# jcasal-homer/HomerHEVC

Hardware: AMD Instinct MI355X
Metric: encoded frames/sec, 1080p & 2160p YUV420 fixed-QP IPPP, 1/2/4/8 MI355X (higher is better)
Workload: dtype int16; 1 GPU; cfg2-1080p-encode; sequences_per_gpu=256, width=1920, height=1080, wfpp_num_threads=17, qp=32, gop=IPPP intra_period=100

## Files before the change

### homerhevc_amd/csrc/enc/enc_common.h

```cpp
#pragma once
#include "enc_prims.h"
#if !defined(__HIPCC__)
#include <stdio.h>
#include <stdlib.h>
#endif

#if !defined(__HIPCC__) && defined(HENC_TRACE_ENABLE)
#include <stdio.h>
extern "C" FILE *henc_trace_file;
#define HENC_TRACE(...) do { if (henc_trace_file) fprintf(henc_trace_file, __VA_ARGS__); } while (0)
#define HENC_TRACE_PW(e, tag)                                                                                                                      \
	do {                                                                                                                                       \
		if (henc_trace_file) {                                                                                                             \
			unsigned a_[3] = {0, 0, 0};                                                                                                \
			for (int c_ = 0; c_ < 3; c_++) {                                                                                           \
				const int n_ = c_ ? 32 : 64;                                                                                       \
				const pred_t *p_ = c_ ? (e).w->pred_c[c_ - 1] : (e).w->pred_y;                                                     \
				for (int y_ = 0; y_ < n_; y_++)                                                                                    \
					for (int x_ = 0; x_ < n_; x_++) a_[c_] += (unsigned)(p_[y_ * n_ + x_] & 0xffff) * (unsigned)(1 + ((x_ + 3 * y_) & 7)); \
			}                                                                                                                          \
			fprintf(henc_trace_file, "PW %s ctu=%d pred=%u,%u,%u\n", tag, (e).ctu->ctu_number, a_[0], a_[1], a_[2]);                   \
		}                                                                                                                                  \
	} while (0)
#else
#define HENC_TRACE(...) do { } while (0)
#define HENC_TRACE_PW(e, tag) do { } while (0)
#endif

enum { PF_SETUP = 0, PF_MERGE, PF_ME_INT, PF_ME_SUB, PF_PRED_INTER, PF_ENC_INTER, PF_INTRA_SEARCH, PF_INTRA_TU, PF_INTRA_CHROMA, PF_CONSOLIDATE, PF_WAIT, PF_TOTAL, PF_PRIM0, PF_COUNT = PF_PRIM0 + 2 * PP_COUNT + 2 };
#if defined(__HIPCC__) && defined(HENC_PROFILE)
#define HENC_PROF_T0() const unsigned long long prof_t0_ = __builtin_amdgcn_s_memtime()
#if defined(HENC_QPROF)
#define HENC_PROF_ADD(e, cat) do { if ((cat) == PF_TOTAL && (e).prof && threadIdx.x == 0) (e).prof[cat] += __builtin_amdgcn_s_memtime() - prof_t0_; } while (0)
#define HENC_QPROF_T0() unsigned long long qprof_t_ = __builtin_amdgcn_s_memtime()
#define HENC_QPROF_MARK(e, cat) do { const unsigned long long now_ = __builtin_amdgcn_s_memtime(); if ((e).prof && threadIdx.x == 0) (e).prof[cat] += now_ - qprof_t_; qprof_t_ = now_; } while (0)
#define HENC_QPROF_ARG , unsigned long long &qprof_t_
#define HENC_QPROF_PASS , qprof_t_
#else
#define HENC_PROF_ADD(e, cat) do { if ((e).prof && threadIdx.x == 0) (e).prof[cat] += __builtin_amdgcn_s_memtime() - prof_t0_; } while (0)
#endif
#else
#define HENC_PROF_T0() do { } while (0)
#define HENC_PROF_ADD(e, cat) do { } while (0)
#endif
#if !defined(HENC_QPROF_MARK)
#define HENC_QPROF_T0() do { } while (0)
#define HENC_QPROF_MARK(e, cat) do { } while (0)
#define HENC_QPROF_ARG
#define HENC_QPROF_PASS
#endif

namespace henc {

#if defined(__HIPCC__)
extern __constant__ Geo henc_geo_table[NNODES];
#endif
#if defined(__HIP_DEVICE_COMPILE__)
struct GeoTable {
	const Geo *p;
	__device__ __forceinline__ const Geo &operator[](int i) const { return henc_geo_table[__builtin_amdgcn_readfirstlane(i)]; }
	__device__ __forceinline__ const Geo &lane(int i) const { return henc_geo_table[i]; }
};
#else
struct GeoTable {
	const Geo *p;
	HENC_INLINE const Geo &operator[](int i) const { return p[i]; }
	HENC_INLINE const Geo &lane(int i) const { return p[i]; }
};
#endif

constexpr int NHELP_MAX = 3;
constexpr int NODES_RESIDENT = 21, NODES_D3 = 85, NODE_QUAD_D3 = 16, NODE_QUAD_D4 = 64, NODE_SLOTS = NODES_RESIDENT + NODE_QUAD_D3 + NODE_QUAD_D4;
// ... 40 lines not shown
	uint32_t inter_ssq[3];
	int inter_ssq_valid;
	int ctu_x, ctu_y;
	uint32_t nb_ctus;
	unsigned long long *timeline;
	int n_spec_reads, n_ratio_cmp, last_slog;
	int n_stale_pred;
	const uint8_t *rd_ctx;
	int rd_luma_depth;
	uint32_t rd_chroma_state;
	HENC_AT(Node, LDS_OFF_NODES) nodes;
	Node *nodes_fast;
	int node_quad;
	HENC_AT(struct HelperBox, LDS_OFF_BOX) box;
	FastPtr<int16_t> adi_c;
	FastPtr<int16_t> mc_tmp_y;
	int mc_tmp_y_stride;
	FastPtr<int16_t> mc_tmp_c;
	FastPtr<int16_t> scratch_a, scratch_b;
	int hseq[NHELP_MAX];
	int bgseq, bg_node;
};

enum { HJOB_NONE = 0, HJOB_NEW_CTU, HJOB_INTER_TU, HJOB_INTRA_SAD, HJOB_SYNC_CU, HJOB_SSD, HJOB_CHROMA_SEARCH, HJOB_CHROMA_TU, HJOB_QUAD_C, HJOB_QUIT };
#if !defined(HENC_NHELP)
#define HENC_NHELP 1
#endif
constexpr int NHELP = HENC_NHELP;
static_assert(NHELP == NHELP_ && (NHELP == 1 || NHELP == 2), "one helper for both chroma planes, or one per plane");
constexpr int COMP_UV = 3;
struct HelperBox {
	int cmd[NHELP], done[NHELP];
	int job[NHELP];
	int a[NHELP][8];
	uint32_t r[NHELP][8];
	int bg_cmd, bg_done, bg_cancel, bg_ni, bg_depth, bg_mode, bg_bits;
};
#if defined(__HIP_DEVICE_COMPILE__)
static_assert(sizeof(HelperBox) <= LDS_BOX_BYTES && sizeof(Enc) <= LDS_ENC_BYTES, "the places of the mailbox and of the contexts in a worker's LDS");
#endif

template <class G>
HENC_HD void helper_post(const G g, Enc &__restrict__ e, int h, int job, int a0 = 0, int a1 = 0, int a2 = 0, int a3 = 0, int a4 = 0, int a5 = 0)
{
	HENC_ENC_IN_LDS(e);
#if defined(__HIP_DEVICE_COMPILE__)
	HelperBox *b = e.box;
// ... 394 lines not shown
```

### homerhevc_amd/csrc/enc/enc_intra.h

```cpp
#pragma once
#include "enc_common.h"
#include "enc_rdo.h"

namespace henc {

HENC_INLINE int intra_is_filtered(int mode, int inv_depth)
{
	static constexpr int intra_filter[5] = {10, 7, 1, 0, 10};
	const int diff = hmin(habs(mode - HOR_IDX), habs(mode - VER_IDX));
	return (mode != DC_IDX) && (diff > intra_filter[inv_depth - 2]);
}

template <class G>
HENC_HD void node_fill_refs(const G g, Enc &__restrict__ e, int ni, int wnd, int comp, int want_filtered)
{
	HENC_ENC_IN_LDS(e);
	const Geo &q = e.geo[ni];
	const Node &nd = node_of(e, ni);
	const int is_y = comp == COMP_Y;
	const int n = is_y ? q.size : q.size_chroma, x = is_y ? q.x : q.xc, y = is_y ? q.y : q.yc;
	const int pw = is_y ? e.seq->width : e.seq->width >> 1, ph = is_y ? e.seq->height : e.seq->height >> 1;
	const int cx = is_y ? e.ctu_x : e.ctu_x >> 1, cy = is_y ? e.ctu_y : e.ctu_y >> 1;
	const int bl_size = hmin(n, ph - (cy + y + n)), tr_size = hmin(n, pw - (cx + x + n));
	const int st = dec_stride(comp);
// ... 30 lines not shown
}
HENC_INLINE void intra_neighbour_dirs(Enc &__restrict__ e, int ni, int depth, int *dirs, uint16_t *src)
{
	HENC_ENC_IN_LDS(e);
	uint32_t idx = 0;
	CtuPublic *cl = pu_left(e, ni, &idx);
	dirs[0] = dirs[1] = DC_IDX;
	src[0] = src[1] = DC_IDX;
	if (cl == e.ctu) { if (e.w->thread_seen_intra) dirs[0] = read_mode_buff(e, depth, idx, &src[0]); }
	else if (cl) src[0] = (uint16_t)(dirs[0] = cl->pred_mode[idx] == PM_INTRA ? cl->intra_mode[COMP_Y][idx] : DC_IDX);
	CtuPublic *ct = pu_top(e, ni, &idx, 1);
	if (ct == e.ctu) { if (e.w->thread_seen_intra) dirs[1] = read_mode_buff(e, depth, idx, &src[1]); }
	else if (ct) src[1] = (uint16_t)(dirs[1] = ct->pred_mode[idx] == PM_INTRA ? ct->intra_mode[COMP_Y][idx] : DC_IDX);
}

template <class SadsFn, class BitsFn>
HENC_INLINE int intra_search_walk_batched(const int *preds, int rd_fast, double sqrt_lambda, SadsFn &&sads_of, int *best_mode_out, double *best_cost_out, BitsFn &&full_bits_of,
					  int *modes_buf = nullptr, int64_t *sads_buf = nullptr)
{
	static constexpr int search_points[4][5] = {{0, 1, 0, 8, 16}, {2, 10, 16, 22, 30}, {-4, -2, 2, 4, 0}, {-1, 1, 0, 0, 0}};
	static constexpr int num_search_points[4] = {2, 5, 4, 2};
	int best_cu_mode = 0, new_best = 0, min_mode = 0, max_mode = 1, best_bit_cost = 0;
	double best_cost = MAX_COST;
	for (int loop = 0; loop < 4; loop++) {
		if (loop == 1) { best_cu_mode = 2; min_mode = 2; max_mode = 34; }
		int modes_local[5], cnt = 0;
		int64_t sads_local[5];
		int *modes = modes_buf ? modes_buf : modes_local;
		int64_t *sads = sads_buf ? sads_buf : sads_local;
		for (int k = 0; k < num_search_points[loop]; k++) {
			const int mode = best_cu_mode + search_points[loop][k];
			if (mode < min_mode || mode > max_mode) continue;
			modes[cnt++] = mode;
		}
		if (!sads_of(modes, cnt, sads)) return -1;
		for (int k = 0; k < cnt; k++) {
			const int mode = modes[k];
			double cost = (double)(uint32_t)sads[k];
			int bit_cost = 0;
			if (rd_fast == 1) {
				bit_cost = (preds[0] == mode || preds[1] == mode || preds[2] == mode) ? 1 : 12;
				cost += bit_cost * sqrt_lambda;
			} else if (rd_fast == 2) {
				bit_cost = (preds[0] == mode || preds[1] == mode || preds[2] == mode) ? (int)full_bits_of(mode) : 6;
				cost += bit_cost * sqrt_lambda;
			}
			if (cost < best_cost) { best_cost = cost; new_best = mode; best_bit_cost = bit_cost; }
		}
		best_cu_mode = new_best;
	}
	*best_mode_out = best_cu_mode;
	*best_cost_out = best_cost;
	return best_bit_cost;
}
template <class SadFn>
HENC_INLINE int intra_search_walk(const int *preds, int rd_fast, double sqrt_lambda, SadFn &&sad_of, int *best_mode_out, double *best_cost_out)
{
	return intra_search_walk_batched(preds, rd_fast, sqrt_lambda, [&](const int *modes, int cnt, int64_t *sads) -> bool {
		for (int k = 0; k < cnt; k++) {
			sads[k] = sad_of(modes[k]);
			if (sads[k] < 0) return false;
		}
		return true;
	}, best_mode_out, best_cost_out, [](int) { return 0u; });
}

HENC_INLINE uint32_t intra_luma_cost(uint32_t tu_cost, int mode_bits, double correction) { return (uint32_t)(tu_cost + mode_bits * correction + .5); }

template <class G>
HENC_HD int intra_mode_search(const G g, Enc &__restrict__ e, int ni, int depth, int *best_mode_out, double *best_cost_out)
{
	HENC_ENC_IN_LDS(e);
	const Geo &q = e.geo[ni];
	Work &w = *e.w;
	const int n = q.size, curr_depth = q.depth, inv_depth = CFG_MAX_CU_SHIFT - curr_depth;
	node_fill_refs(g, e, ni, depth + 1, COMP_Y, 1);
	int preds[3], dirs[2];
	uint16_t src[2];
	e.rd_luma_depth = curr_depth;
	intra_neighbour_dirs(e, ni, curr_depth, dirs, src);
	mpm_from_dirs(dirs[0], dirs[1], preds);
	const int rd_fast = e.seq->rd_mode == RDM_FAST ? 1 : (rd_full(g, *e.seq) ? 2 : 0);
	SearchLog *lg = nullptr;
	e.last_slog = -1;
	if (rd_fast == 1 && ((src[0] | src[1]) & 0x8000)) {
		if (e.n_spec_reads < MAX_SEARCH_LOGS) {
			lg = e.ctu_g->slog + e.n_spec_reads;
			lg->src[0] = src[0]; lg->src[1] = src[1];
			lg->used[0] = (uint8_t)dirs[0]; lg->used[1] = (uint8_t)dirs[1];
			lg->n = 0;
			lg->has_cmp = 0;
			lg->tu_cost = 0;
			e.last_slog = e.n_spec_reads;
		}
		e.n_spec_reads++;
	}
	const src_t *orig = w.curr_y + q.y * CTU_STRIDE_Y + q.x;
	return intra_search_walk_batched(preds, rd_fast, e.f->sqrt_lambda, [&](const int *modes, int cnt, int64_t *sads) -> bool {
		for (int k0 = 0; k0 < cnt;) {
			const int take = HENC_HELPERS(e) ? hmin(1 + NHELP, cnt - k0) : 1, mine = k0 + take - 1;
			for (int j = 0; j < take - 1; j++) helper_post(g, e, j, HJOB_INTRA_SAD, ni, n, modes[k0 + j], intra_is_filtered(modes[k0 + j], inv_depth));
			{
				const int mode = modes[mine], filt = intra_is_filtered(mode, inv_depth);
				sads[mine] = (int64_t)intra_predict_sad(g, (pred_t *)nullptr, 0, orig, CTU_STRIDE_Y, filt ? w.adi_f : w.adi, n, mode, 1);
			}
			for (int j = 0; j < take - 1; j++) {
				helper_wait(g, e, j);
				sads[k0 + j] = (int64_t)e.box->r[j][0];
			}
			k0 += take;
		}
		if (lg)
			for (int k = 0; k < cnt; k++) {
				lg->mode[lg->n] = (uint8_t)modes[k];
				lg->sad[lg->n] = (uint32_t)sads[k];
				lg->n++;
			}
		return true;
	}, best_mode_out, best_cost_out, [&](int mode) { return rd_bits_luma_mode_in_preds(e, mode, preds); }, w.srch_modes, w.srch_sads);
}

template <class G>
HENC_HD void set_intra_info_buffs(const G g, Enc &__restrict__ e, int depth, int ni)
{
	HENC_ENC_IN_LDS(e);
	const Geo &q = e.geo[ni];
	const Node &nd = node_of(e, ni);
	Work &w = *e.w;
	for (int i = g.tid; i < q.num_part; i += g.n) {
		w.cbf_buffs[COMP_Y][depth][q.abs_index + i] = (uint8_t)nd.intra_cbf[COMP_Y];
		w.tr_idx_buffs[depth][q.abs_index + i] = (uint8_t)nd.intra_tr_idx;
		w.intra_mode_buffs[COMP_Y][depth][q.abs_index + i] = (uint8_t)nd.intra_mode[COMP_Y];
	}
	g.sync();
}

template <class G>
HENC_HD uint32_t encode_intra_tu(const G g, Enc &__restrict__ e, int ni, int depth, int cu_mode, int part_size_type, int *curr_sum)
{
	HENC_ENC_IN_LDS(e);
	const Geo &q = e.geo[ni];
	Node &nd = node_of(e, ni);
// ... 202 lines not shown
		return intra_luma_cost(tn.cost, bitcost_cu_mode, correction);
	}
	return tn.cost;
}

HENC_INLINE void chroma_dir_list(int *list, int luma_mode)
{
	list[0] = PLANAR_IDX; list[1] = VER_IDX; list[2] = HOR_IDX; list[3] = DC_IDX; list[4] = DM_CHROMA_IDX;
#pragma unroll
	for (int i = 0; i < 4; i++)
		if (luma_mode == list[i]) list[i] = 34;
}

template <class G>
HENC_WALK_FN HENC_HD void chroma_search_comp(const G g, Enc &__restrict__ e, int curr, int c, const int *cand, uint32_t *sads)
{
	HENC_ENC_IN_LDS(e);
	Work &w = *e.w;
	const Geo &q = e.geo[curr];
	const int n = q.size_chroma;
	pred_t *pred = pred_ptr(w, c) + q.yc * CTU_STRIDE_C + q.xc;
	const src_t *orig = curr_ptr(w, c) + q.yc * CTU_STRIDE_C + q.xc;
	node_fill_refs(g, e, curr, NWND - 1, c, 0);
	for (int mi = 0; mi < 5; mi++) sads[mi] = intra_predict_sad(g, pred, CTU_STRIDE_C, orig, CTU_STRIDE_C, e.adi_c, n, cand[mi], 0);
}
template <class G>
HENC_HD int chroma_tu_comp(const G g, Enc &__restrict__ e, int curr, int c, int cu_mode, int scan_mode, int shifts, int per, int rem, int *curr_sum_out)
{
	HENC_ENC_IN_LDS(e);
	Work &w = *e.w;
	const Geo &q = e.geo[curr];
	const int n = q.size_chroma, curr_depth = q.depth, qwnd = NWND - 1, dwnd = NWND - 1;
	pred_t *pred = pred_ptr(w, c) + q.yc * CTU_STRIDE_C + q.xc;
	const src_t *orig = curr_ptr(w, c) + q.yc * CTU_STRIDE_C + q.xc;
	int16_t *quant = tq_ptr(w, qwnd, c) + ((q.abs_index << 4) >> 2), *iquant = iq_slot(w, c, (q.abs_index << 4) >> 2, e.on_helper);
	int16_t *dec = dec_ptr(w, dwnd, c) + q.yc * DEC_STRIDE_C + q.xc;
	node_fill_refs(g, e, curr, dwnd, c, 0);
	intra_predict(g, pred, CTU_STRIDE_C, e.adi_c, n, cu_mode, 0);
	tr_forward(g, HENC_FT(e), e.T, orig, CTU_STRIDE_C, pred, CTU_STRIDE_C, e.scratch_a, e.scratch_b, n, 0);
	const int curr_sum = quantize(g, HENC_FT(e), e.T, e.scratch_a, iquant, e.scratch_b, scan_mode, curr_depth, c, 1, e.f->slice_type == SLICE_I, e.seq->sign_hiding, n, per, rem);
	const int cbfv = ((curr_sum ? 1 : 0) << (shifts & 255)) | ((curr_sum ? 1 : 0) << (shifts >> 8));
	bytes_set(g, &w.cbf_chroma[c - 1][q.abs_index], cbfv, q.num_part);
	uint32_t raw;
	if (curr_sum) {
		lin_copy_nosync(g, iquant, quant, n * n);
		dequantize(g, HENC_FT(e), e.T, iquant, iquant, curr_depth, c, 1, n, per, rem);
		tr_inverse(g, HENC_FT(e), e.T, e.scratch_b, n, iquant, e.scratch_a, n, 0);
// ... 32 lines not shown
	} else parent = e.geo[curr].parent;
	const int luma_mode = w.intra_mode_buffs[COMP_Y][depth][e.geo[curr].abs_index];
#if !defined(__HIPCC__)
	if (luma_mode & MODE_TOKEN) { fprintf(stderr, "encode_intra_chroma: inherited luma mode\n"); abort(); }
#endif
	int mode_list[5];
	chroma_dir_list(mode_list, luma_mode);
	if (e.geo[curr].size_chroma == 2) {
		curr = parent;
		parent = e.geo[curr].parent;
	}
	int best_modes[3] = {0, 0, 0};
	double best_costs[3] = {1.7e+308, 1.7e+308, 1.7e+308};
	uint32_t best_bits[3] = {0, 0, 0};
	{
		const Geo &q = e.geo[curr];
		const int n = q.size_chroma;
		uint32_t sad_u[5], sad_v[5];
		int cand[5];
#pragma unroll
		for (int mi = 0; mi < 5; mi++) cand[mi] = mode_list[mi] == DM_CHROMA_IDX ? luma_mode : mode_list[mi];
		if (HENC_HELPERS(e)) {
			helper_post(g, e, 0, HJOB_CHROMA_SEARCH, curr, COMP_U, cand[0] | (cand[1] << 8) | (cand[2] << 16) | (cand[3] << 24), cand[4]);
			chroma_search_comp(g, e, curr, COMP_V, cand, sad_v);
			helper_wait(g, e, 0);
#pragma unroll
			for (int mi = 0; mi < 5; mi++) sad_u[mi] = e.box->r[0][mi];
		} else {
			chroma_search_comp(g, e, curr, COMP_U, cand, sad_u);
			chroma_search_comp(g, e, curr, COMP_V, cand, sad_v);
		}
#pragma unroll
		for (int mi = 0; mi < 5; mi++) {
			uint32_t distortion = sad_u[mi], cost = distortion;
			distortion += sad_v[mi];
			cost += distortion;
			uint32_t bit_cost = mode_list[mi] == DM_CHROMA_IDX ? 1 : 12;
			if (rd_full(g, S)) {
				const Geo &sq = e.geo[curr];
				bytes_set(g, &w.intra_mode_buffs[COMP_CHR][depth][sq.abs_index], mode_list[mi], sq.num_part);
				RdViews &rv = rd_views_of(e);
				rd_make_views(g, e, rv, depth, depth, nullptr, nullptr, depth, nullptr, nullptr, nullptr);
				bit_cost = rd_bits_chroma_mode(e, rv.v, curr);
			}
			cost += (uint32_t)(bit_cost * e.f->sqrt_lambda + .5);
			int um = mode_list[mi];
			double uc = cost;
			uint32_t ub = bit_cost;
#pragma unroll
			for (int i = 0; i < 3; i++)
				if (best_costs[i] > uc) {
					const int am = best_modes[i]; const double ac = best_costs[i]; const uint32_t ab = best_bits[i];
					best_costs[i] = uc; best_modes[i] = um; best_bits[i] = ub;
// ... 131 lines not shown
```

### homerhevc_amd/csrc/enc/enc_prims.h

```cpp
#pragma once
#include "enc_types.h"
#include "../tables_layout.h"

enum { PP_SAD = 0, PP_SSD, PP_BLK, PP_FILLREF, PP_ADIFILT, PP_INTRAPRED, PP_INTERP, PP_TRF, PP_TRI, PP_QUANT, PP_DEQUANT, PP_CAND, PP_SYNC, PP_INFO, PP_CTU_IO, PP_HWAIT, PP_COUNT };
#if defined(__HIPCC__) && defined(HENC_PROFILE)
extern __shared__ __align__(16) unsigned char henc_lds[];
#define HENC_LDS_PROF_OFFSET 43008
#define PRIM_T0() const unsigned long long prim_t0_ = __builtin_amdgcn_s_memtime()
#define PRIM_END(cat) do { if (threadIdx.x == 0) { unsigned long long *pp_ = (unsigned long long *)(henc_lds + HENC_LDS_PROF_OFFSET); pp_[cat] += __builtin_amdgcn_s_memtime() - prim_t0_; pp_[PP_COUNT + (cat)]++; } } while (0)
#else
#define PRIM_T0() do { } while (0)
#define PRIM_END(cat) do { } while (0)
#endif

namespace henc {

HENC_INLINE int ilog2i(int n)
{
	return n <= 1 ? 0 : 32 - __builtin_clz((unsigned)(n - 1));
}
HENC_INLINE void split_rc(int k, int w, int lw, int *r, int *c)
{
	if ((w & (w - 1)) == 0) { *r = k >> lw; *c = k & (w - 1); }
	else { *r = k / w; *c = k - *r * w; }
// ... 560 lines not shown
	PRIM_END(PP_INTRAPRED);
}

template <class G, class S, class P>
HENC_PRIM uint32_t intra_predict_sad(const G g, P *pred, int ps, const S *orig, int os, const int16_t *adi, int n, int mode, int is_luma)
{
	PRIM_T0();
	if constexpr (G::n == 64) { mode = uni(mode); n = uni(n); is_luma = uni(is_luma); }
	const IntraPredictor p = intra_setup(g, adi, n, mode, is_luma);
	const int l = p.shift;
	uint32_t acc = 0;
	#pragma unroll 4
	for (int k = g.tid; k < n * n; k += g.n) {
		const int j = k >> l, i = k & (n - 1);
		const int v = intra_sample(p, j, i);
		if (pred) pred[j * ps + i] = (P)v;
		acc += (uint32_t)habs((int16_t)(orig[j * os + i] - (int16_t)v));
	}
	const uint32_t s = g.sum(acc);
	g.sync();
	{ const auto prim_ret_ = s; PRIM_END(PP_INTRAPRED); return prim_ret_; }
}

HENC_INLINE void luma_tap_row(int f, int *c)
{
	const int t[4][8] = {{0, 0, 0, 64, 0, 0, 0, 0}, {-1, 4, -10, 58, 17, -5, 1, 0}, {-1, 4, -11, 40, 40, -11, 4, -1}, {0, 1, -5, 17, 58, -10, 4, -1}};
	for (int k = 0; k < 8; k++) c[k] = t[f][k];
}
HENC_INLINE void chroma_tap_row(int f, int *c)
{
	const int t[8][4] = {{0, 64, 0, 0}, {-2, 58, 10, -2}, {-4, 54, 16, -2}, {-6, 46, 28, -4}, {-4, 36, 36, -4}, {-4, 28, 46, -6}, {-2, 16, 54, -4}, {-2, 10, 58, -2}};
	for (int k = 0; k < 4; k++) c[k] = t[f][k];
}

template <int NT, class G>
HENC_PRIM void interp_stage(const G g, const int16_t *src, int ss, int16_t *dst, int ds, int fraction, int w, int h, int vert, int first, int last)
{
	PRIM_T0();
	if (NT == 4 && w < 4 && fraction == 0) { g.sync(); PRIM_END(PP_INTERP); return; }
	const int lw = ilog2i(w);
	if ((w & 3) != 0 || (fraction != 0 && w * h < 4 * G::n && G::n > 1)) {
		int c8[8];
		if (NT == 8) luma_tap_row(fraction, c8);
		else chroma_tap_row(fraction, c8);
		const int rs = vert ? ss : 1;
		int shift = 6, offset;
// ... 807 lines not shown
```

### homerhevc_amd/csrc/enc/enc_types.h

```cpp
#pragma once
#include "enc_platform.h"

namespace henc {

enum { COMP_Y = 0, COMP_U = 1, COMP_V = 2, COMP_CHR = 1 };
enum { PM_INTER = 0, PM_INTRA = 1 };
enum { PART_2Nx2N = 0, PART_NxN = 3 };
enum { SLICE_B = 0, SLICE_P = 1, SLICE_I = 2 };
enum { RDM_DIST_ONLY = 0, RDM_FULL = 1, RDM_FAST = 2 };
enum { ME_PEL = 1, ME_HALF = 2, ME_QUARTER = 4 };
enum { PLANAR_IDX = 0, DC_IDX = 1, HOR_IDX = 10, VER_IDX = 26, DM_CHROMA_IDX = 36, REG_DCT = 65535 };
enum { SCAN_ZIGZAG = 0, SCAN_HOR = 1, SCAN_VER = 2, SCAN_DIAG = 3 };

constexpr int NPART = 256;
constexpr int NNODES = 341;
constexpr int NDEPTH = 5;
constexpr int NWND = 7;
constexpr uint32_t MAX_COST = 0xffffffffu / 8;

constexpr int MAX_SEARCH_LOGS = 192, MAX_RATIO_CMP = 96;
constexpr int POST_MAX_ROWS = 128;
constexpr int HENC_MAX_STEPS = 192;
constexpr int MODE_TOKEN = 0x80;

// ... 157 lines not shown
#if defined(__HIPCC__)
	int16_t iq_y[32 * 32], iq_c[HENC_IQ_SLOTS][32 * 32];
#else
	int16_t iq_y[64 * 64], iq_c[2][32 * 32];
#endif
	uint8_t cbf_buffs[3][NDEPTH][NPART];
	uint8_t intra_mode_buffs[2][NDEPTH][NPART];
#if defined(__HIPCC__)
	const uint8_t (*mode_in)[NDEPTH][NPART];
#else
	uint8_t mode_in[2][NDEPTH][NPART];
#endif
	uint8_t tr_idx_buffs[NDEPTH][NPART];
	uint8_t cbf_chroma[2][NPART];
	int16_t adi[264], adi_f[264];
	int16_t pred_aux[TU_SCRATCH];
	int16_t delta_u[TU_SCRATCH];
#if !defined(__HIPCC__)
	int16_t sub_tmp[(64 + 8) * 72];
#endif
	MvCandList amvp, merge_cands, search_cands;
	uint32_t rsplit[11];
	uint32_t pad_rsplit_;
	alignas(8) int64_t srch_sads[5];
	int32_t srch_modes[6];
#if !defined(__HIPCC__)
	uint8_t nodes_fast_store[52 * (21 + 16 + 64) + 16];
#endif
	HENC_GLOBAL_PTR(WorkSlow) slow;
	int32_t thread_seen_intra;
#if !defined(__HIPCC__)
	struct WorkRd *rd_store;
#endif
};
struct WorkRd {
	uint8_t rd_pred_depth[NPART], rd_part_size[NPART], rd_pred_mode[NPART], rd_luma_modes[NPART];
	uint8_t rd_ctx_work[RD_CTX_BYTES];
	EntScratch rd_ent;
	alignas(8) unsigned char rd_views[512];
};

HENC_INLINE int16_t *wnd_y(int16_t *base) { return base; }

HENC_INLINE int16_t *dec_ptr(Work &w, int wnd, int comp)
{
	return (int16_t *)(comp == COMP_Y ? w.slow->dec_y[wnd] + DEC_ORG_Y : w.slow->dec_c[wnd][comp - 1] + DEC_ORG_C);
}
HENC_INLINE int dec_stride(int comp) { return comp == COMP_Y ? DEC_STRIDE_Y : DEC_STRIDE_C; }
// ... 18 lines not shown
```

### homerhevc_amd/csrc/k_encode.hip

```cpp
#define HENC_TU_OPERANDS_IN_LDS 1
#include <stddef.h>
#include <stdlib.h>
#include <algorithm>
#include <chrono>
#include <mutex>
#include <condition_variable>
#include <new>
#include <string>
#include <thread>
#include <vector>

#include <type_traits>
#include "common.h"
#include "enc/enc_sched.h"
#include "enc/enc_host.h"
#include "enc/enc_post.h"
#include "picture_io.h"

using namespace henc;

int hmr_subpel_plane_on(hipStream_t stream, int comp, const int16_t *pic, int stride, int rows, uint8_t *out);
int hmr_subpel_planes_on(hipStream_t stream, const int16_t *pic_y, const int16_t *pic_u, const int16_t *pic_v, int stride_y, int rows_y, int stride_c, int rows_c, uint8_t *out_y,
			 uint8_t *out_u, uint8_t *out_v);

// ... 139 lines not shown
			const Geo &q = e.geo[a[0]];
			if (a[1] == COMP_UV) {
				const int n = q.size_chroma, l = ilog2i(n);
				uint32_t acc[2] = {0, 0};
				for (int i = g.tid * 4; i < n * n; i += 64 * 4) {
					const int o = q.yc * 32 + q.xc + (i >> l) * 32 + (i & (n - 1));
#pragma unroll
					for (int c = 0; c < 2; c++) {
						const S4 va = ld4(e.w->curr_c[c] + o), vb = ld4(e.w->pred_c[c] + o);
#pragma unroll
						for (int k = 0; k < 4; k++) { const int32_t dd = (int16_t)(va.v[k] - vb.v[k]); acc[c] += (uint32_t)(dd * dd); }
					}
				}
				r0 = g.sum(acc[0]);
				r1 = g.sum(acc[1]);
			} else {
				const int c = a[1] - 1;
				r0 = blk_ssd(g, e.w->curr_c[c] + q.yc * 32 + q.xc, 32, e.w->pred_c[c] + q.yc * 32 + q.xc, 32, q.size_chroma);
			}
			break;
		}
		case HJOB_CHROMA_SEARCH: {
			const int cand[5] = {a[2] & 255, (a[2] >> 8) & 255, (a[2] >> 16) & 255, (a[2] >> 24) & 255, a[3]};
			uint32_t sads[5];
			chroma_search_comp(g, e, a[0], a[1], cand, sads);
			g.sync();
			if (g.tid == 0)
				for (int k = 0; k < 5; k++) box->r[h][k] = sads[k];
			break;
		}
		case HJOB_CHROMA_TU: {
			int cs = 0;
			r0 = (uint32_t)chroma_tu_comp(g, e, a[0], a[1], a[2], a[3], a[4], a[5] & 255, a[5] >> 8, &cs);
			r1 = (uint32_t)cs;
			break;
		}
#if defined(HENC_QUAD)
		case HJOB_QUAD_C:
			quad_chroma_job(g, e, a[0], a[1]);
			break;
#endif
		case HJOB_INTRA_SAD: {
			const Geo &q = e.geo[a[0]];
			r0 = intra_predict_sad(g, (pred_t *)nullptr, 0, e.w->curr_y + q.y * CTU_STRIDE_Y + q.x, CTU_STRIDE_Y, a[3] ? e.w->adi_f : e.w->adi, a[1], a[2], 1);
			break;
		}
		default: break;
		}
		g.sync();
		if (g.tid == 0) {
			if (job != HJOB_CHROMA_SEARCH) { box->r[h][0] = r0; box->r[h][1] = r1; box->r[h][2] = r2; box->r[h][3] = r3; box->r[h][4] = r4; box->r[h][5] = r5; }
			__hip_atomic_store(&box->done[h], seq, __ATOMIC_RELEASE, __HIP_MEMORY_SCOPE_WORKGROUP);
		}
	}
	return true;
}

__device__ __attribute__((noinline)) bool helper_serve_out(HelperBox *box, int h, int16_t *scratch, const WaveGrp g, int seq) { return helper_serve(box, h, scratch, g, seq); }

__device__ __attribute__((noinline)) bool helper_bg_search(HelperBox *box, int h, int16_t *scratch, const WaveGrp g, int &seq, int bgseq)
{
	extern __shared__ __align__(16) uint8_t lds[];
	Enc &e = *(Enc *)(lds + LDS_OFF_ENC + (1 + h) * LDS_ENC_BYTES);
	HENC_ENC_IN_LDS(e);
	const int ni = uni(box->bg_ni), depth = uni(box->bg_depth);
	const Geo &q = e.geo[ni];
	const int n = q.size, curr_depth = q.depth, inv_depth = CFG_MAX_CU_SHIFT - curr_depth;
	bool quit = false;
	int best_mode = 0, bits = -1;
	double best_cost = 0;
	if (__hip_atomic_load(&box->bg_cancel, __ATOMIC_ACQUIRE, __HIP_MEMORY_SCOPE_WORKGROUP) != bgseq) {
		node_fill_refs(g, e, ni, depth + 1, COMP_Y, 1);
		int preds[3], dirs[2];
		uint16_t src[2];
// ... 634 lines not shown
```

### homerhevc_amd/csrc/k_primtest.hip

```cpp
#include <stdlib.h>
#include <string.h>
#include <vector>

#include "common.h"
#include "enc/enc_prims.h"

using namespace henc;

hmr_gpu_ctx *hmr_default_ctx();

namespace {

enum { PT_SAD = 1, PT_SSD, PT_PREDICT, PT_RECONST, PT_VARIANCE, PT_INTRA_PRED, PT_FILL_REFS, PT_ADI_FILTER, PT_TRANSFORM, PT_ITRANSFORM, PT_QUANT, PT_INV_QUANT };

struct PtArgs {
	int op, bytes;
	int p[12];
	long off[6];
};

int g_bytes = 0;

__global__ __launch_bounds__(64) void k_primtest(PtArgs a, int16_t *arena, uint8_t *arena8, const DevTables *T, uint32_t *ret)
{
	const WaveGrp g{(int)threadIdx.x};
	const int *p = a.p;
	auto A = [&](int k) { return arena + a.off[k]; };
	auto B = [&](int k) { return arena8 + a.off[k]; };
	uint32_t r = 0;
	switch (a.op) {
	case PT_SAD: r = blk_sad(g, A(0), p[0], A(1), p[1], p[2]); break;
	case PT_SSD: r = a.bytes ? blk_ssd(g, B(0), p[0], B(1), p[1], p[2]) : blk_ssd(g, A(0), p[0], A(1), p[1], p[2]); break;
	case PT_PREDICT:
		if (a.bytes) blk_predict(g, B(0), p[0], B(1), p[1], A(2), p[2], p[3]);
		else blk_predict(g, A(0), p[0], A(1), p[1], A(2), p[2], p[3]);
		break;
	case PT_RECONST: {
		const int16_t *res = p[1] ? A(1) : nullptr;
		if (a.bytes) blk_reconst(g, B(0), p[0], res, p[1], A(2), p[2], p[3]);
		else blk_reconst(g, A(0), p[0], res, p[1], A(2), p[2], p[3]);
		break;
	}
	case PT_VARIANCE: r = a.bytes ? blk_modified_variance(g, B(0), p[1], p[0], p[2]) : blk_modified_variance(g, A(0), p[1], p[0], p[2]); break;
	case PT_INTRA_PRED:
		if (a.bytes) {
			intra_predict(g, B(0), p[0], A(1), p[1], p[2], p[3]);
			g.sync();
			for (int i = g.tid; i < p[1] * p[1]; i += 64) A(0)[(i / p[1]) * p[0] + i % p[1]] = B(0)[(i / p[1]) * p[0] + i % p[1]];
		} else intra_predict(g, A(0), p[0], A(1), p[1], p[2], p[3]);
		break;
	case PT_FILL_REFS: intra_fill_refs(g, A(0), p[0], p[1], p[2], p[3], p[4], p[5], p[6], p[7], A(1)); break;
	case PT_ADI_FILTER: intra_adi_filter(g, A(0), A(1), p[0], p[1]); break;
	case PT_TRANSFORM:
		if (a.bytes) tr_forward(g, (const FastTables *)nullptr, T, B(0), p[0], B(3), p[0], A(1), A(2), p[1], p[2]);
		else tr_forward(g, (const FastTables *)nullptr, T, A(0), p[0], A(3), p[0], A(1), A(2), p[1], p[2]);
		break;
	case PT_ITRANSFORM: tr_inverse(g, (const FastTables *)nullptr, T, A(0), p[0], A(1), A(2), p[1], p[2]); break;
	case PT_QUANT: r = (uint32_t)quantize(g, (const FastTables *)nullptr, T, A(0), A(1), A(2), p[0], p[1], p[2], p[3], p[4], p[5], p[6], p[7], p[8]); break;
	case PT_INV_QUANT: dequantize(g, (const FastTables *)nullptr, T, A(0), A(1), p[0], p[1], p[2], p[3], p[4], p[5]); break;
	default: break;
	}
	g.sync();
	if (g.tid == 0) *ret = r;
}

struct Operand {
	const int16_t *in;
	int16_t *out;
	size_t elems;
};

uint32_t run(int op, const int *p, int np, Operand *ops, int nops)
{
	hmr_gpu_ctx *c = hmr_default_ctx();
	if (!c) { fprintf(stderr, "hmr_gpu_prim_*: no device\n"); abort(); }
	PtArgs a;
	memset(&a, 0, sizeof a);
	a.op = op;
	a.bytes = g_bytes;
	for (int i = 0; i < np; i++) a.p[i] = p[i];
	size_t total = 0;
	for (int k = 0; k < nops; k++) {
// ... 140 lines not shown
	}
	Operand ops[4] = {{block, nullptr, span(block_stride, n, n)}, {nullptr, coeff, (size_t)n * n}, {nullptr, nullptr, (size_t)n * n}, {nullptr, nullptr, span(block_stride, n, n)}};
	const int p[3] = {block_stride, n, is_dst};
	run(PT_TRANSFORM, p, 3, ops, 4);
}
void hmr_gpu_prim_itransform(int16_t *block, int16_t *coeff, int block_stride, int n, int is_dst)
{
	Operand ops[3] = {{block, block, span(block_stride, n, n)}, {coeff, nullptr, (size_t)n * n}, {nullptr, nullptr, (size_t)n * n}};
	const int p[3] = {block_stride, n, is_dst};
	run(PT_ITRANSFORM, p, 3, ops, 3);
}
void hmr_gpu_prim_quant(int16_t *src, int16_t *dst, int16_t *delta_u, int scan_mode, int depth, int comp, int is_intra, int slice_is_intra, int sign_hiding, int *ac_sum,
			int cu_size, int per, int rem)
{
	Operand ops[3] = {{src, nullptr, (size_t)cu_size * cu_size}, {nullptr, dst, (size_t)cu_size * cu_size}, {nullptr, delta_u, (size_t)cu_size * cu_size}};
	const int p[9] = {scan_mode, depth, comp, is_intra, slice_is_intra, sign_hiding, cu_size, per, rem};
	*ac_sum = (int)run(PT_QUANT, p, 9, ops, 3);
}
void hmr_gpu_prim_inv_quant(int16_t *src, int16_t *dst, int depth, int comp, int is_intra, int cu_size, int per, int rem)
{
	Operand ops[2] = {{src, nullptr, (size_t)cu_size * cu_size}, {nullptr, dst, (size_t)cu_size * cu_size}};
	const int p[6] = {depth, comp, is_intra, cu_size, per, rem};
	run(PT_INV_QUANT, p, 6, ops, 2);
}
int hmr_gpu_prim_multi_sad(int maxc, const uint8_t *src, const uint8_t *plane, size_t plane_bytes, const int64_t *cand_off, int ncalls, int stride, int n, uint32_t *out)
{
	if (!src || !plane || !cand_off || !out || ncalls < 1 || ncalls > 65536 || (maxc != 4 && maxc != 8 && maxc != 9) || (n != 8 && n != 16 && n != 32 && n != 64) || stride < 1) {
		hmr_set_error("hmr_gpu_prim_multi_sad: maxc 4 / 8 / 9, n 8 / 16 / 32 / 64, a stride of at least 1, 1 .. 65536 lists");
		return HMR_GPU_ERR_ARG;
	}
	for (int i = 0; i < ncalls * maxc; i++) {
		const int64_t o = cand_off[i];
		if (o == -1) continue;
		if (o < 0 || (uint64_t)o + (uint64_t)(n - 1) * (uint64_t)stride + (uint64_t)n > (uint64_t)plane_bytes) {
			hmr_set_error("hmr_gpu_prim_multi_sad: candidate %d of list %d does not lie inside the plane", i % maxc, i / maxc);
			return HMR_GPU_ERR_ARG;
		}
	}
	hmr_gpu_ctx *c = hmr_default_ctx();
	if (!c) { hmr_set_error("hmr_gpu_prim_multi_sad: no device"); return HMR_GPU_ERR_NO_DEVICE; }
	HIP_TRY(hipSetDevice(c->device));
	struct Bufs {
		void *p[4] = {nullptr, nullptr, nullptr, nullptr};
		~Bufs() { for (void *q : p) if (q) (void)hipFree(q); }
	} b;
	const size_t nres = (size_t)ncalls * maxc;
// ... 17 lines not shown
```

### include/homer_gpu.h

```cpp
#ifndef HOMER_GPU_H
#define HOMER_GPU_H

#include <stddef.h>
#include <stdint.h>

#ifdef __cplusplus
extern "C" {
#endif

typedef struct hmr_gpu_ctx hmr_gpu_ctx;

enum hmr_gpu_status {
	HMR_GPU_OK = 0,
	HMR_GPU_ERR_NO_DEVICE = -1,
	HMR_GPU_ERR_HIP = -2,
	HMR_GPU_ERR_ARG = -3,
	HMR_GPU_ERR_NOMEM = -4
};


int hmr_gpu_create(hmr_gpu_ctx **out, int device, void *stream);
void hmr_gpu_destroy(hmr_gpu_ctx *ctx);
const char *hmr_gpu_last_error(void);
int hmr_gpu_sync(hmr_gpu_ctx *ctx);
// ... 439 lines not shown

int hmr_gpu_subpel_planes(hmr_gpu_ctx *ctx, const int16_t *pic_y, const int16_t *pic_u, const int16_t *pic_v, int stride_y, int rows_y, int stride_c, int rows_c,
			  uint8_t *out_y, uint8_t *out_u, uint8_t *out_v);

int hmr_gpu_probe_valu_issue(hmr_gpu_ctx *ctx, int waves_per_simd, int dependent, double *wave_instr_per_s, double *ms);
int hmr_gpu_probe_issue(hmr_gpu_ctx *ctx, int op, int waves_per_simd, int dependent, double *wave_instr_per_s, double *ms);

void hmr_gpu_prim_bytes(int on);
uint32_t hmr_gpu_prim_sad(int16_t *src, uint32_t src_stride, int16_t *pred, uint32_t pred_stride, int size);
uint32_t hmr_gpu_prim_ssd16b(int16_t *src, uint32_t src_stride, int16_t *pred, uint32_t pred_stride, int size);
void hmr_gpu_prim_predict(int16_t *orig, int orig_stride, int16_t *pred, int pred_stride, int16_t *residual, int residual_stride, int size);
void hmr_gpu_prim_reconst(int16_t *pred, int pred_stride, int16_t *residual, int residual_stride, int16_t *decoded, int decoded_stride, int size);
uint32_t hmr_gpu_prim_modified_variance(int16_t *p, int size, int stride, int modif);
void hmr_gpu_prim_intra_planar(int16_t *prediction, int pred_stride, int16_t *adi_pred_buff, int adi_size, int cu_size);
void hmr_gpu_prim_intra_angular(int16_t *prediction, int pred_stride, int16_t *adi_pred_buff, int adi_size, int cu_size, int cu_mode, int is_luma);
void hmr_gpu_prim_fill_reference_samples(int16_t *decoded_corner, int stride, int n, int left, int top, int bottom_left, int top_right, int bl_size, int tr_size, int16_t *adi);
void hmr_gpu_prim_adi_filter(int16_t *adi, int16_t *out, int adi_size, int n, int strong_enabled);
void hmr_gpu_prim_transform(int16_t *block, int16_t *coeff, int block_stride, int n, int is_dst);
void hmr_gpu_prim_itransform(int16_t *block, int16_t *coeff, int block_stride, int n, int is_dst);
void hmr_gpu_prim_quant(int16_t *src, int16_t *dst, int16_t *delta_u, int scan_mode, int depth, int comp, int is_intra, int slice_is_intra, int sign_hiding, int *ac_sum,
			int cu_size, int per, int rem);
void hmr_gpu_prim_inv_quant(int16_t *src, int16_t *dst, int depth, int comp, int is_intra, int cu_size, int per, int rem);
int hmr_gpu_prim_multi_sad(int maxc, const uint8_t *src, const uint8_t *plane, size_t plane_bytes, const int64_t *cand_off, int ncalls, int stride, int n, uint32_t *out);

enum hmr_gpu_walk_step { HMR_GPU_WALK_QUAD8_Y = 1, HMR_GPU_WALK_QUAD8_C, HMR_GPU_WALK_QUAD16_Y, HMR_GPU_WALK_QUAD16_C, HMR_GPU_WALK_TU, HMR_GPU_WALK_TU_PAIR };
typedef struct hmr_gpu_walk_case {
	int32_t step, node, comp, one_slot;
	int32_t qp, ctu_x, ctu_y, slice_type;
	int32_t sign_hiding, chroma_qp_offset, stride_y, stride_c;
	int32_t mv[4][2];
	double avg_dist, chroma_weight;
	int64_t sub_y, sub_c[2], curr, pred;
} hmr_gpu_walk_case;
typedef struct hmr_gpu_walk_out {
	uint32_t dist[4][3];
	int32_t sum[4][3];
	uint32_t raw[4][3], cbf[4][3];
	uint32_t stray, reserved[15];
	uint8_t pred[4][256];
	int16_t rec[4][256], lv[4][256];
} hmr_gpu_walk_out;
int hmr_gpu_walk_forms(const hmr_gpu_walk_case *cases, int ncases, const uint8_t *arena, size_t arena_bytes, hmr_gpu_walk_out *out);

#ifdef __cplusplus
}
#endif
// ... 2 lines not shown
```

Baseline: 493.1 frames/s.

## Batch intra direction SADs into one multi-mode primitive and split across helper

Adds a multi-direction intra predict+SAD primitive that keeps the source block in registers and reduces all directions at the end, rather than one predict/SAD with its own reduction and sync per mode. The luma search merges the first two search stages into one batch of up to seven modes and sends half the batch to a helper wave in a single mailbox post, replacing the per-mode helper handshakes. Chroma search uses the same batched primitive. The cost is speculative SAD work for the second-stage modes, higher register pressure from the accumulators, and extra profiling macros and a test entry point.

New measurement: 487.5 frames/s. -1.1%, worse.

```diff
diff --git a/homerhevc_amd/csrc/enc/enc_common.h b/homerhevc_amd/csrc/enc/enc_common.h
--- a/homerhevc_amd/csrc/enc/enc_common.h
+++ b/homerhevc_amd/csrc/enc/enc_common.h
@@ -33,7 +33,14 @@
 #if defined(HENC_QPROF)
 #define HENC_PROF_ADD(e, cat) do { if ((cat) == PF_TOTAL && (e).prof && threadIdx.x == 0) (e).prof[cat] += __builtin_amdgcn_s_memtime() - prof_t0_; } while (0)
 #define HENC_QPROF_T0() unsigned long long qprof_t_ = __builtin_amdgcn_s_memtime()
-#define HENC_QPROF_MARK(e, cat) do { const unsigned long long now_ = __builtin_amdgcn_s_memtime(); if ((e).prof && threadIdx.x == 0) (e).prof[cat] += now_ - qprof_t_; qprof_t_ = now_; } while (0)
+#define HENC_QPROF_MARK_(e, cat) do { const unsigned long long now_ = __builtin_amdgcn_s_memtime(); if ((e).prof && threadIdx.x == 0) (e).prof[cat] += now_ - qprof_t_; qprof_t_ = now_; } while (0)
+#if HENC_QPROF == 2
+#define HENC_QPROF_MARK(e, cat) do { (void)qprof_t_; } while (0)
+#define HENC_IQPROF_MARK(e, cat) HENC_QPROF_MARK_(e, cat)
+#define HENC_IQPROF_COUNT(e, cat, k) do { if ((e).prof && threadIdx.x == 0) (e).prof[cat] += (k); } while (0)
+#else
+#define HENC_QPROF_MARK(e, cat) HENC_QPROF_MARK_(e, cat)
+#endif
 #define HENC_QPROF_ARG , unsigned long long &qprof_t_
 #define HENC_QPROF_PASS , qprof_t_
 #else
@@ -48,6 +55,10 @@
 #define HENC_QPROF_MARK(e, cat) do { } while (0)
 #define HENC_QPROF_ARG
 #define HENC_QPROF_PASS
+#endif
+#if !defined(HENC_IQPROF_MARK)
+#define HENC_IQPROF_MARK(e, cat) do { } while (0)
+#define HENC_IQPROF_COUNT(e, cat, k) do { } while (0)
 #endif
 
 namespace henc {
@@ -134,7 +145,8 @@
 	int bgseq, bg_node;
 };
 
-enum { HJOB_NONE = 0, HJOB_NEW_CTU, HJOB_INTER_TU, HJOB_INTRA_SAD, HJOB_SYNC_CU, HJOB_SSD, HJOB_CHROMA_SEARCH, HJOB_CHROMA_TU, HJOB_QUAD_C, HJOB_QUIT };
+enum { HJOB_NONE = 0, HJOB_NEW_CTU, HJOB_INTER_TU, HJOB_INTRA_SAD, HJOB_SYNC_CU, HJOB_SSD, HJOB_CHROMA_SEARCH, HJOB_CHROMA_TU, HJOB_QUAD_C, HJOB_QUIT,
+       HJOB_INTRA_SADS };
 #if !defined(HENC_NHELP)
 #define HENC_NHELP 1
 #endif
diff --git a/homerhevc_amd/csrc/enc/enc_intra.h b/homerhevc_amd/csrc/enc/enc_intra.h
--- a/homerhevc_amd/csrc/enc/enc_intra.h
+++ b/homerhevc_amd/csrc/enc/enc_intra.h
@@ -76,19 +76,27 @@
 	static constexpr int num_search_points[4] = {2, 5, 4, 2};
 	int best_cu_mode = 0, new_best = 0, min_mode = 0, max_mode = 1, best_bit_cost = 0;
 	double best_cost = MAX_COST;
+	int modes_local[7], cnt = 0, first = 0;
+	int64_t sads_local[7];
+	int *modes = modes_buf ? modes_buf : modes_local;
+	int64_t *sads = sads_buf ? sads_buf : sads_local;
 	for (int loop = 0; loop < 4; loop++) {
 		if (loop == 1) { best_cu_mode = 2; min_mode = 2; max_mode = 34; }
-		int modes_local[5], cnt = 0;
-		int64_t sads_local[5];
-		int *modes = modes_buf ? modes_buf : modes_local;
-		int64_t *sads = sads_buf ? sads_buf : sads_local;
-		for (int k = 0; k < num_search_points[loop]; k++) {
-			const int mode = best_cu_mode + search_points[loop][k];
-			if (mode < min_mode || mode > max_mode) continue;
-			modes[cnt++] = mode;
-		}
-		if (!sads_of(modes, cnt, sads)) return -1;
-		for (int k = 0; k < cnt; k++) {
+		if (loop == 1) { first = cnt; cnt += num_search_points[1]; }
+		else {
+			first = cnt = 0;
+			for (int k = 0; k < num_search_points[loop]; k++) {
+				const int mode = best_cu_mode + search_points[loop][k];
+				if (mode < min_mode || mode > max_mode) continue;
+				modes[cnt++] = mode;
+			}
+			const int mine = cnt;
+			if (loop == 0)
+				for (int k = 0; k < num_search_points[1]; k++) modes[cnt++] = 2 + search_points[1][k];
+			if (!sads_of(modes, cnt, sads)) return -1;
+			cnt = mine;
+		}
+		for (int k = first; k < cnt; k++) {
 			const int mode = modes[k];
 			double cost = (double)(uint32_t)sads[k];
 			int bit_cost = 0;
@@ -128,7 +136,9 @@
 	const Geo &q = e.geo[ni];
 	Work &w = *e.w;
 	const int n = q.size, curr_depth = q.depth, inv_depth = CFG_MAX_CU_SHIFT - curr_depth;
+	HENC_QPROF_T0();
 	node_fill_refs(g, e, ni, depth + 1, COMP_Y, 1);
+	HENC_IQPROF_MARK(e, 1);
 	int preds[3], dirs[2];
 	uint16_t src[2];
 	e.rd_luma_depth = curr_depth;
@@ -150,20 +160,32 @@
 		e.n_spec_reads++;
 	}
 	const src_t *orig = w.curr_y + q.y * CTU_STRIDE_Y + q.x;
-	return intra_search_walk_batched(preds, rd_fast, e.f->sqrt_lambda, [&](const int *modes, int cnt, int64_t *sads) -> bool {
-		for (int k0 = 0; k0 < cnt;) {
-			const int take = HENC_HELPERS(e) ? hmin(1 + NHELP, cnt - k0) : 1, mine = k0 + take - 1;
-			for (int j = 0; j < take - 1; j++) helper_post(g, e, j, HJOB_INTRA_SAD, ni, n, modes[k0 + j], intra_is_filtered(modes[k0 + j], inv_depth));
-			{
-				const int mode = modes[mine], filt = intra_is_filtered(mode, inv_depth);
-				sads[mine] = (int64_t)intra_predict_sad(g, (pred_t *)nullptr, 0, orig, CTU_STRIDE_Y, filt ? w.adi_f : w.adi, n, mode, 1);
-			}
-			for (int j = 0; j < take - 1; j++) {
-				helper_wait(g, e, j);
-				sads[k0 + j] = (int64_t)e.box->r[j][0];
-			}
-			k0 += take;
-		}
+	HENC_IQPROF_MARK(e, 2);
+	HENC_IQPROF_COUNT(e, 7, 1);
+	const int bits = intra_search_walk_batched(preds, rd_fast, e.f->sqrt_lambda, [&](const int *modes, int cnt, int64_t *sads) -> bool {
+		#if defined(HENC_INTRA_SPLIT_FIRST_ONLY)
+		const int theirs = HENC_HELPERS(e) && cnt == INTRA_SADS_MAX ? cnt >> 1 : 0, mine = cnt - theirs;
+#else
+		const int theirs = HENC_HELPERS(e) ? cnt >> 1 : 0, mine = cnt - theirs;
+#endif
+		HENC_IQPROF_MARK(e, 6);
+		HENC_IQPROF_COUNT(e, 8, 1);
+		HENC_IQPROF_COUNT(e, 9, cnt);
+		uint64_t list = 0;
+#pragma unroll
+		for (int k = 0; k < INTRA_SADS_MAX; k++) {
+			const int mode = modes[k];
+			list |= (uint64_t)(k < cnt ? intra_sads_entry(mode, intra_is_filtered(mode, inv_depth)) : 0u) << (8 * k);
+		}
+		if (theirs) helper_post(g, e, 0, HJOB_INTRA_SADS, ni, n, (int)(uint32_t)(list >> (8 * mine)), theirs);
+		HENC_IQPROF_MARK(e, 3);
+		intra_predict_sads(g, (pred_t *)nullptr, 0, orig, CTU_STRIDE_Y, (const int16_t *)w.adi, (const int16_t *)w.adi_f, n, list, mine, 1, sads);
+		HENC_IQPROF_MARK(e, 4);
+		if (theirs) {
+			helper_wait(g, e, 0);
+			for (int j = 0; j < theirs; j++) sads[mine + j] = (int64_t)e.box->r[0][j];
+		}
+		HENC_IQPROF_MARK(e, 5);
 		if (lg)
 			for (int k = 0; k < cnt; k++) {
 				lg->mode[lg->n] = (uint8_t)modes[k];
@@ -172,6 +194,8 @@
 			}
 		return true;
 	}, best_mode_out, best_cost_out, [&](int mode) { return rd_bits_luma_mode_in_preds(e, mode, preds); }, w.srch_modes, w.srch_sads);
+	HENC_IQPROF_MARK(e, 6);
+	return bits;
 }
 
 template <class G>
@@ -420,7 +444,10 @@
 	pred_t *pred = pred_ptr(w, c) + q.yc * CTU_STRIDE_C + q.xc;
 	const src_t *orig = curr_ptr(w, c) + q.yc * CTU_STRIDE_C + q.xc;
 	node_fill_refs(g, e, curr, NWND - 1, c, 0);
-	for (int mi = 0; mi < 5; mi++) sads[mi] = intra_predict_sad(g, pred, CTU_STRIDE_C, orig, CTU_STRIDE_C, e.adi_c, n, cand[mi], 0);
+	uint64_t list = 0;
+#pragma unroll
+	for (int mi = 0; mi < 5; mi++) list |= (uint64_t)intra_sads_entry(cand[mi], 0) << (8 * mi);
+	intra_predict_sads(g, pred, CTU_STRIDE_C, orig, CTU_STRIDE_C, (const int16_t *)e.adi_c, (const int16_t *)e.adi_c, n, list, 5, 0, sads);
 }
 template <class G>
 HENC_HD int chroma_tu_comp(const G g, Enc &__restrict__ e, int curr, int c, int cu_mode, int scan_mode, int shifts, int per, int rem, int *curr_sum_out)
@@ -499,13 +526,17 @@
 		for (int mi = 0; mi < 5; mi++) cand[mi] = mode_list[mi] == DM_CHROMA_IDX ? luma_mode : mode_list[mi];
 		if (HENC_HELPERS(e)) {
 			helper_post(g, e, 0, HJOB_CHROMA_SEARCH, curr, COMP_U, cand[0] | (cand[1] << 8) | (cand[2] << 16) | (cand[3] << 24), cand[4]);
-			chroma_search_comp(g, e, curr, COMP_V, cand, sad_v);
+			chroma_search_comp(g, e, curr, COMP_V, cand, w.srch_out);
 			helper_wait(g, e, 0);
 #pragma unroll
-			for (int mi = 0; mi < 5; mi++) sad_u[mi] = e.box->r[0][mi];
+			for (int mi = 0; mi < 5; mi++) { sad_u[mi] = e.box->r[0][mi]; sad_v[mi] = w.srch_out[mi]; }
 		} else {
-			chroma_search_comp(g, e, curr, COMP_U, cand, sad_u);
-			chroma_search_comp(g, e, curr, COMP_V, cand, sad_v);
+			chroma_search_comp(g, e, curr, COMP_U, cand, w.srch_out);
+#pragma unroll
+			for (int mi = 0; mi < 5; mi++) sad_u[mi] = w.srch_out[mi];
+			chroma_search_comp(g, e, curr, COMP_V, cand, w.srch_out);
+#pragma unroll
+			for (int mi = 0; mi < 5; mi++) sad_v[mi] = w.srch_out[mi];
 		}
 #pragma unroll
 		for (int mi = 0; mi < 5; mi++) {
diff --git a/homerhevc_amd/csrc/enc/enc_prims.h b/homerhevc_amd/csrc/enc/enc_prims.h
--- a/homerhevc_amd/csrc/enc/enc_prims.h
+++ b/homerhevc_amd/csrc/enc/enc_prims.h
@@ -606,6 +606,65 @@
 	{ const auto prim_ret_ = s; PRIM_END(PP_INTRAPRED); return prim_ret_; }
 }
 
+constexpr int INTRA_SADS_MAX = 7;
+HENC_INLINE uint32_t intra_sads_entry(int mode, int filtered) { return (uint32_t)mode | (filtered ? 128u : 0u); }
+template <class G, class S, class P, class O>
+#if defined(__HIPCC__) && defined(HENC_INTRA_SADS_OUTLINE)
+__device__ __attribute__((noinline))
+#elif defined(__HIPCC__)
+__device__ __forceinline__
+#else
+inline
+#endif
+void intra_predict_sads(const G g, P *pred, int ps, const S *orig, int os, const int16_t *adi, const int16_t *adi_f, int n, uint64_t list, int cnt, int is_luma, O *out)
+{
+	PRIM_T0();
+	uint32_t list_lo = (uint32_t)list, list_hi = (uint32_t)(list >> 32);
+	if constexpr (G::n == 64) {
+		pred = uni_ptr(pred); orig = uni_ptr(orig); adi = uni_ptr(adi); adi_f = uni_ptr(adi_f); out = uni_ptr(out);
+		ps = uni(ps); os = uni(os); n = uni(n); cnt = uni(cnt); is_luma = uni(is_luma); list_lo = uni(list_lo); list_hi = uni(list_hi);
+	}
+	HENC_OP_IN_LDS(orig); HENC_OP_IN_LDS(adi); HENC_OP_IN_LDS(adi_f); HENC_OP_IN_LDS(out);
+	cnt = hmin(cnt, INTRA_SADS_MAX);
+	const int l = ilog2i(n), total = n * n;
+	const bool kept = total <= 4 * G::n;
+	uint64_t src4 = 0;
+	if (kept) {
+#pragma unroll
+		for (int t = 0; t < 4; t++) {
+			const int k = g.tid + t * G::n;
+			if (k < total) src4 |= (uint64_t)(uint16_t)orig[(k >> l) * os + (k & (n - 1))] << (16 * t);
+		}
+	}
+	uint32_t acc[INTRA_SADS_MAX];
+#pragma unroll
+	for (int j = 0; j < INTRA_SADS_MAX; j++) acc[j] = 0;
+#pragma unroll 1
+	for (int d = 0; d < cnt; d++) {
+		const uint32_t ent = ((d < 4 ? list_lo >> (8 * d) : list_hi >> (8 * (d - 4))) & 255u);
+		const IntraPredictor p = intra_setup(g, (ent & 128u) ? adi_f : adi, n, (int)(ent & 127u), is_luma);
+		const bool store = pred != nullptr && d == cnt - 1;
+		uint32_t s = 0;
+		#pragma unroll 4
+		for (int k = g.tid, t = 0; k < total; k += G::n, t++) {
+			const int j = k >> l, i = k & (n - 1);
+			const int v = intra_sample(p, j, i);
+			if (store) pred[j * ps + i] = (P)v;
+			const int o = kept ? (int)(int16_t)(src4 >> (16 * (t & 3))) : (int)orig[j * os + i];
+			s += (uint32_t)habs((int16_t)(o - (int16_t)v));
+		}
+#pragma unroll
+		for (int j = 0; j < INTRA_SADS_MAX; j++) acc[j] = d == j ? s : acc[j];
+	}
+#pragma unroll
+	for (int j = 0; j < INTRA_SADS_MAX; j++) {
+		const uint32_t sum = g.sum(acc[j]);
+		if (j < cnt) out[j] = (O)sum;
+	}
+	g.sync();
+	PRIM_END(PP_INTRAPRED);
+}
+
 HENC_INLINE void luma_tap_row(int f, int *c)
 {
 	const int t[4][8] = {{0, 0, 0, 64, 0, 0, 0, 0}, {-1, 4, -10, 58, 17, -5, 1, 0}, {-1, 4, -11, 40, 40, -11, 4, -1}, {0, 1, -5, 17, 58, -10, 4, -1}};
diff --git a/homerhevc_amd/csrc/enc/enc_types.h b/homerhevc_amd/csrc/enc/enc_types.h
--- a/homerhevc_amd/csrc/enc/enc_types.h
+++ b/homerhevc_amd/csrc/enc/enc_types.h
@@ -203,8 +203,9 @@
 	MvCandList amvp, merge_cands, search_cands;
 	uint32_t rsplit[11];
 	uint32_t pad_rsplit_;
-	alignas(8) int64_t srch_sads[5];
-	int32_t srch_modes[6];
+	alignas(8) int64_t srch_sads[7];
+	int32_t srch_modes[8];
+	uint32_t srch_out[8];
 #if !defined(__HIPCC__)
 	uint8_t nodes_fast_store[52 * (21 + 16 + 64) + 16];
 #endif
diff --git a/homerhevc_amd/csrc/k_encode.hip b/homerhevc_amd/csrc/k_encode.hip
--- a/homerhevc_amd/csrc/k_encode.hip
+++ b/homerhevc_amd/csrc/k_encode.hip
@@ -185,11 +185,12 @@
 		}
 		case HJOB_CHROMA_SEARCH: {
 			const int cand[5] = {a[2] & 255, (a[2] >> 8) & 255, (a[2] >> 16) & 255, (a[2] >> 24) & 255, a[3]};
-			uint32_t sads[5];
-			chroma_search_comp(g, e, a[0], a[1], cand, sads);
-			g.sync();
-			if (g.tid == 0)
-				for (int k = 0; k < 5; k++) box->r[h][k] = sads[k];
+			chroma_search_comp(g, e, a[0], a[1], cand, box->r[h]);
+			break;
+		}
+		case HJOB_INTRA_SADS: {
+			const Geo &q = e.geo[a[0]];
+			intra_predict_sads(g, (pred_t *)nullptr, 0, e.w->curr_y + q.y * CTU_STRIDE_Y + q.x, CTU_STRIDE_Y, (const int16_t *)e.w->adi, (const int16_t *)e.w->adi_f, a[1], (uint64_t)(uint32_t)a[2], a[3], 1, box->r[h]);
 			break;
 		}
 		case HJOB_CHROMA_TU: {
@@ -212,7 +213,7 @@
 		}
 		g.sync();
 		if (g.tid == 0) {
-			if (job != HJOB_CHROMA_SEARCH) { box->r[h][0] = r0; box->r[h][1] = r1; box->r[h][2] = r2; box->r[h][3] = r3; box->r[h][4] = r4; box->r[h][5] = r5; }
+			if (job != HJOB_CHROMA_SEARCH && job != HJOB_INTRA_SADS) { box->r[h][0] = r0; box->r[h][1] = r1; box->r[h][2] = r2; box->r[h][3] = r3; box->r[h][4] = r4; box->r[h][5] = r5; }
 			__hip_atomic_store(&box->done[h], seq, __ATOMIC_RELEASE, __HIP_MEMORY_SCOPE_WORKGROUP);
 		}
 	}
diff --git a/homerhevc_amd/csrc/k_primtest.hip b/homerhevc_amd/csrc/k_primtest.hip
--- a/homerhevc_amd/csrc/k_primtest.hip
+++ b/homerhevc_amd/csrc/k_primtest.hip
@@ -11,7 +11,7 @@
 
 namespace {
 
-enum { PT_SAD = 1, PT_SSD, PT_PREDICT, PT_RECONST, PT_VARIANCE, PT_INTRA_PRED, PT_FILL_REFS, PT_ADI_FILTER, PT_TRANSFORM, PT_ITRANSFORM, PT_QUANT, PT_INV_QUANT };
+enum { PT_SAD = 1, PT_SSD, PT_PREDICT, PT_RECONST, PT_VARIANCE, PT_INTRA_PRED, PT_FILL_REFS, PT_ADI_FILTER, PT_TRANSFORM, PT_ITRANSFORM, PT_QUANT, PT_INV_QUANT, PT_INTRA_SADS };
 
 struct PtArgs {
 	int op, bytes;
@@ -58,6 +58,24 @@
 	case PT_ITRANSFORM: tr_inverse(g, (const FastTables *)nullptr, T, A(0), p[0], A(1), A(2), p[1], p[2]); break;
 	case PT_QUANT: r = (uint32_t)quantize(g, (const FastTables *)nullptr, T, A(0), A(1), A(2), p[0], p[1], p[2], p[3], p[4], p[5], p[6], p[7], p[8]); break;
 	case PT_INV_QUANT: dequantize(g, (const FastTables *)nullptr, T, A(0), A(1), p[0], p[1], p[2], p[3], p[4], p[5]); break;
+	case PT_INTRA_SADS: {
+		uint32_t *out = (uint32_t *)A(3);
+		const uint64_t list = (uint64_t)(uint32_t)p[4] | ((uint64_t)(uint32_t)p[5] << 32);
+		if (p[6]) {
+			for (int k = 0; k < p[3]; k++) {
+				const int ent = (int)((list >> (8 * k)) & 255);
+				const uint32_t s = a.bytes ? intra_predict_sad(g, (uint8_t *)nullptr, 0, B(0), p[0], ent & 128 ? A(2) : A(1), p[1], ent & 127, p[2])
+							   : intra_predict_sad(g, (int16_t *)nullptr, 0, A(0), p[0], ent & 128 ? A(2) : A(1), p[1], ent & 127, p[2]);
+				if (g.tid == 0) out[k] = s;
+			}
+		} else if (a.bytes) {
+			intra_predict_sads(g, p[7] ? B(4) : (uint8_t *)nullptr, p[7], B(0), p[0], A(1), A(2), p[1], list, p[3], p[2], out);
+			g.sync();
+			if (p[7])
+				for (int i = g.tid; i < p[1] * p[1]; i += 64) A(4)[(i / p[1]) * p[7] + i % p[1]] = B(4)[(i / p[1]) * p[7] + i % p[1]];
+		} else intra_predict_sads(g, p[7] ? A(4) : (int16_t *)nullptr, p[7], A(0), p[0], A(1), A(2), p[1], list, p[3], p[2], out);
+		break;
+	}
 	default: break;
 	}
 	g.sync();
@@ -244,6 +262,27 @@
 	Operand ops[2] = {{src, nullptr, (size_t)cu_size * cu_size}, {nullptr, dst, (size_t)cu_size * cu_size}};
 	const int p[6] = {depth, comp, is_intra, cu_size, per, rem};
 	run(PT_INV_QUANT, p, 6, ops, 2);
+}
+int hmr_gpu_prim_intra_sads(const int16_t *orig, int orig_stride, const int16_t *adi, const int16_t *adi_f, int n, const int *modes, const int *filtered, int count, int is_luma, int single,
+			    uint32_t *sads, int16_t *last_pred)
+{
+	if (!orig || !adi || !adi_f || !modes || !filtered || !sads || (n != 4 && n != 8 && n != 16 && n != 32) || orig_stride < n || count < 1 || count > INTRA_SADS_MAX) {
+		hmr_set_error("hmr_gpu_prim_intra_sads: n 4 / 8 / 16 / 32, a source stride of at least n, 1 .. %d directions", INTRA_SADS_MAX);
+		return HMR_GPU_ERR_ARG;
+	}
+	uint64_t list = 0;
+	for (int k = 0; k < count; k++) {
+		if (modes[k] < 0 || modes[k] > 34) { hmr_set_error("hmr_gpu_prim_intra_sads: direction %d", modes[k]); return HMR_GPU_ERR_ARG; }
+		list |= (uint64_t)intra_sads_entry(modes[k], filtered[k]) << (8 * k);
+	}
+	if (!hmr_default_ctx()) { hmr_set_error("hmr_gpu_prim_intra_sads: no device"); return HMR_GPU_ERR_NO_DEVICE; }
+	int16_t res[2 * 8];
+	memset(res, 0, sizeof res);
+	Operand ops[5] = {{orig, nullptr, span(orig_stride, n, n)}, {adi, nullptr, (size_t)(4 * n + 1)}, {adi_f, nullptr, (size_t)(4 * n + 1)}, {res, res, 16}, {nullptr, last_pred, (size_t)n * n}};
+	const int p[8] = {orig_stride, n, is_luma, count, (int)(uint32_t)list, (int)(uint32_t)(list >> 32), single ? 1 : 0, last_pred && !single ? n : 0};
+	run(PT_INTRA_SADS, p, 8, ops, last_pred ? 5 : 4);
+	memcpy(sads, res, (size_t)count * 4);
+	return HMR_GPU_OK;
 }
 int hmr_gpu_prim_multi_sad(int maxc, const uint8_t *src, const uint8_t *plane, size_t plane_bytes, const int64_t *cand_off, int ncalls, int stride, int n, uint32_t *out)
 {
diff --git a/include/homer_gpu.h b/include/homer_gpu.h
--- a/include/homer_gpu.h
+++ b/include/homer_gpu.h
@@ -485,6 +485,8 @@
 			int cu_size, int per, int rem);
 void hmr_gpu_prim_inv_quant(int16_t *src, int16_t *dst, int depth, int comp, int is_intra, int cu_size, int per, int rem);
 int hmr_gpu_prim_multi_sad(int maxc, const uint8_t *src, const uint8_t *plane, size_t plane_bytes, const int64_t *cand_off, int ncalls, int stride, int n, uint32_t *out);
+int hmr_gpu_prim_intra_sads(const int16_t *orig, int orig_stride, const int16_t *adi, const int16_t *adi_f, int n, const int *modes, const int *filtered, int count, int is_luma, int single,
+                            uint32_t *sads, int16_t *last_pred);
 
 enum hmr_gpu_walk_step { HMR_GPU_WALK_QUAD8_Y = 1, HMR_GPU_WALK_QUAD8_C, HMR_GPU_WALK_QUAD16_Y, HMR_GPU_WALK_QUAD16_C, HMR_GPU_WALK_TU, HMR_GPU_WALK_TU_PAIR };
 typedef struct hmr_gpu_walk_case {
```
